# Lecanyu/SparsifyPoseGraph

Measured on AMD Instinct MI355X. Metric: nodes_marginalized_per_s, higher is better.
Workload: dtype f64

## Files before the change

### sparsifyposegraph_amd/csrc/spg_host_stream.cpp

```cpp
#include "spg_graph_impl.h"

#if defined(__x86_64__)
#include <x86intrin.h>
static inline uint64_t ticks_now() { return __rdtsc(); }
#else
static inline uint64_t ticks_now() { return (uint64_t)(now_s() * 1e9); }
#endif

namespace {
enum : uint8_t { SV_WAITING = 0, SV_STABLE = 1, SV_INFLIGHT = 2, SV_DONE = 3 };
constexpr int kStreamSlots = 2048;
constexpr int kStreamMailStride = 8;

__attribute__((always_inline)) inline void unregister_blanket(spg_graph *g, const int32_t s) {
    const spg_graph::SSlot &sl = g->sslots[s];
    spg_graph::VRec *const vr = g->vr.data();
    for (int i = 0; i < sl.nv; i++) {
        spg_graph::SVtx &sx = vr[sl.verts[i]].s;
        for (int j = 0; j < sx.nown; j++) if (sx.own[j] == s) { sx.own[j] = sx.own[--sx.nown]; break; }
    }
}

struct Streamer {
    spg_graph *g;
    const bool emulate;
    const int D, ps, rec;
    const int32_t P;
    int32_t cursor = 0;
    int32_t prefetched_to = 0;
    int32_t n_done = 0, n_inflight = 0, pending_bell = 0, bell_no = 0;
    bool fallback = false;
    int32_t cap_wait = -1;
    uint64_t t_idle = 0;

    Streamer(spg_graph *g_, bool emu) : g(g_), emulate(emu), D(g_->d), ps(g_->ps), rec(g_->rec), P((int32_t)g_->pending.size()), arena_dev(g_->dev) {}

    struct SvView { spg_graph::VRec *vr; spg_graph::SVtx &operator[](int32_t i) const { return vr[i].s; } };

    long n_exam = 0, n_park[8] = {0};
    const bool prof = [] { const char *e = getenv("SPG_STREAM_PROF"); return e && e[0] == '1'; }();
    uint64_t pt[8] = {0}, pn[8] = {0}, pt_last = 0;
    inline void P0() { if (prof) pt_last = ticks_now(); }
    inline void P1(int i) { if (prof) { const uint64_t n = ticks_now(); pt[i] += n - pt_last; pn[i]++; pt_last = n; } }
    void park(std::vector<int32_t> &heads, int32_t on, int32_t p) { g->wl_next[p] = heads[on]; heads[on] = p; }
    void wake(std::vector<int32_t> &heads, int32_t on) {
        for (int32_t p = heads[on]; p >= 0;) { const int32_t nx = g->wl_next[p]; g->s_woken.push_back(p); p = nx; }
        heads[on] = -1;
    }

    static inline int find(const int32_t *X, const int nX, const int32_t y) { for (int i = 0; i < nX; i++) if (X[i] == y) return i; return -1; }
    static inline void adj_remove(InlVec<spg_graph::AdjEnt, 7> &av, const int32_t eid) {
        for (size_t j = 0; j < av.size(); j++) if (av[j].eid == eid) { av[j] = av.back(); av.pop_back(); break; }
    }
    inline void set_pend(spg_graph::SSlot &sl, const int32_t *X, const int nX) {
        const int32_t *const cst = g->cst.data();
        sl.npend = 0;
        for (int i = 1; i < nX; i++) if (cst[X[i]] >= 0) { if (sl.npend == 3) { sl.npend = -1; break; } sl.pend[sl.npend++] = X[i]; }
    }
    __attribute__((always_inline)) inline void register_blanket(const int32_t s, const int32_t p, const int32_t *X, const int nX) {
        const SvView sv{g->vr.data()};
        spg_graph::SSlot &sl = g->sslots[s];
        sl.pos = p; sl.root = X[0]; sl.nv = nX;
        memcpy(sl.verts, X, sizeof(int32_t) * (size_t)nX);
        set_pend(sl, X, nX);
        for (int i = 0; i < nX; i++) { spg_graph::SVtx &sx = sv[X[i]]; sx.own[sx.nown++] = s; }
    }
// ... 123 lines not shown
        if (mine < 0) {
            for (int i = 0; i < nX; i++) if (sv[X[i]].nown == spg_graph::kSOwn) { park(g->wl_done, slots[sv[X[i]].own[0]].pos, p); return 0; }
            if (g->s_free.empty()) { g->wl_next[p] = cap_wait; cap_wait = p; return 0; }
        }
        if (!emulate && cell_slot[launch_seq & (uint32_t)(port.slots - 1)] != -1) { g->wl_next[p] = cap_wait; cap_wait = p; return 0; }
        const int n_new_max = k - 1, n_new_vert_max = 2 * (k - 1);
        const int64_t new_len = (int64_t)n_new_max * rec, out_len = emulate ? SPG_OUT_LEN(n_new_max, n_new_vert_max) : 0;
        if (g->used + new_len + out_len > g->cap) { fallback = true; return 0; }
        for (int i = 1; i < ne; i++) {
            const int32_t eid = E[i]; const int64_t key = edges[eid].key;
            int j = i - 1;
            for (; j >= 0 && edges[E[j]].key > key; j--) E[j + 1] = E[j];
            E[j + 1] = eid;
        }
        int32_t s = mine;
        if (s < 0) { s = g->s_free.back(); g->s_free.pop_back(); }
        spg_graph::SSlot &sl = g->sslots[s];
        if (mine < 0) register_blanket(s, p, X, nX);
        sl.ne = ne; sl.n_new_max = n_new_max; sl.logi = -1; sl.bell = bell_no + 1; sl.launched = 1;
        sl.tag = (++g->ctx->tag_counter & 0x3fffffff) + 1;
        sl.mcell = (int32_t)(launch_seq & (uint32_t)(port.slots - 1));
        if (!emulate) { cell_slot[sl.mcell] = s; launch_seq++; }
        sl.out_off = emulate ? g->used : -1;
        sl.new_off = g->used + out_len;
        g->used += new_len + out_len;
        memcpy(sl.edges, E, sizeof(int32_t) * (size_t)ne);
        cst[v] = (p << 2) | SV_INFLIGHT; sv[v].slot = s;
        P1(3);
        if (!emulate) build_packet(s, pending_bell);
        if (helper) hp.cell_tag[sl.mcell] = (uint32_t)sl.tag;
        P1(4);
        pending_bell++;
        n_inflight++;
        if (emulate) g->s_fifo.push_back(s);
        if (g->wl_stable[p] >= 0) wake(g->wl_stable, p);
        return 1;
    }

    void commit(const int32_t s, const double *recd, const bool final_seen) {
        spg_graph::SSlot &sl = g->sslots[s];
        const int32_t p = sl.pos, v = sl.root;
        const int status = (int)recd[0], inf = (int)recd[1], n_new = (int)recd[4];
        sl.logi = (int32_t)g->log.size();
        g->log.push_back({g->vid[v], sl.bell, status, inf, recd[2], recd[3]});
        g->stats.max_blanket = std::max(g->stats.max_blanket, sl.nv);
        const bool fine = (status == SPG_OK || status == SPG_ST_KLD_NOT_PD);
        if (!fine) g->stats.n_bad_status++;
        else {
            for (int i = 0; i < sl.ne; i++) {
                const int32_t eid = sl.edges[i];
                GEdge &e = g->edges[eid];
                e.alive = 0;
                adj_remove(g->vr[e.vtx[0]].adj, eid);
                if (e.vtx[1] != e.vtx[0]) adj_remove(g->vr[e.vtx[1]].adj, eid);
            }
            g->n_mutations += sl.ne + 1;
            g->n_live_e -= sl.ne;
            g->valive[v] = 0;
            g->vr[v].adj.clear();
            g->n_live_v--;
            g->stats.n_removed++;
            const int64_t key0 = g->key_base + (int64_t)p * spg_graph::kKeyStride;
            if (!emulate) {
                for_each_compact_edge(recd, n_new, [&](int e, int la, int lb) {
                    const int32_t va = sl.verts[la], vb = sl.verts[lb];
                    GEdge ge;
// ... 257 lines not shown
        std::vector<spg_blanket_desc> blk(take);
        std::vector<int64_t> vpo;
        std::vector<spg_edge_ref> er;
        std::vector<int32_t> ev;
        for (size_t t = 0; t < take; t++) {
            const spg_graph::SSlot &sl = g->sslots[fifo[live[t]]];
            spg_blanket_desc &bd = blk[t];
            append_blanket_desc(g, sl.verts, sl.nv, 1, sl.edges, sl.ne, bd, vpo, er, ev);
            bd.n_new_max = sl.n_new_max; bd.n_new_vert_max = 2 * sl.n_new_max;
            bd.new_off = sl.new_off; bd.new_len = (int64_t)sl.n_new_max * rec; bd.out_off = sl.out_off;
        }
        spg_round_desc rd{};
        rd.opts = &g->opts; rd.n_blankets = (int32_t)take; rd.first = 0; rd.count = (int32_t)take;
        rd.blankets = blk.data(); rd.vert_pose_off = vpo.data(); rd.edges = er.data(); rd.edge_vert = ev.data();
        rd.n_vert_total = (int64_t)vpo.size(); rd.n_edge_total = (int64_t)er.size(); rd.n_edge_vert_total = (int64_t)ev.size();
        rd.mail_base = 0; rd.mail_len = 0; rd.slot = 0; rd.tag = ++g->ctx->tag_counter;
        if (int r = g->ctx->be.run_round(g->ctx->be.user, g->dev, &rd)) return r;
        if (int r = g->ctx->be.synchronize(g->ctx->be.user)) return r;
        for (size_t t = 0; t < take; t++) {
            const int32_t s = fifo[live[t]];
            const spg_graph::SSlot &sl = g->sslots[s];
            const int64_t olen = SPG_OUT_LEN(sl.n_new_max, 2 * sl.n_new_max);
            if (int r = g->ctx->be.download(g->ctx->be.user, g->host.data() + sl.out_off, (char *)g->dev + sl.out_off * 8, olen)) return r;
            ready.push_back(s);
            fifo[live[t]] = -1;
        }
        while (fifo_head < fifo.size() && fifo[fifo_head] < 0) fifo_head++;
        return 0;
    }

    std::vector<int32_t> &woken = g->s_woken, &ready = g->s_ready, &fin = g->s_fin;
    size_t fin_head = 0;
    unsigned n_polls = 0;
    uint64_t last_progress = 0, idle_since = 0;

    int take_results() {
        ready.clear();
        P0();
        if (emulate) { if (int r = poll_emulated()) return r; }
        else if (n_inflight) {
            if (helper) take_helper_results(); else poll_hip((++n_polls & 15) ? 10 : 1 << 20);
        }
        P1(0);
        return 0;
    }
    void commit_ready() {
        for (size_t ri = 0; ri < ready.size(); ri++) {
            const int32_t s = ready[ri];
            const double *recd = emulate ? g->host.data() + g->sslots[s].out_off : (helper ? ready_rec[ri] : cell(s));
            const bool fin_now = emulate || (helper ? (((uint64_t)recd[5]) & 1) != 0 : mail_state(recd[5], g->sslots[s].tag) == MAIL_FINAL);
            P0();
            commit(s, recd, fin_now);
            P1(1);
        }
    }
    void examine_woken() {
        if (!fallback) {
            if (woken.size() > 1) std::sort(woken.begin(), woken.end());
            for (size_t wi = 0; wi < woken.size(); wi++) {
                examine(woken[wi]);
                if (pending_bell >= 8) ring();
            }
        }
        woken.clear();
    }
    void late_results() {
        if (emulate || !(fin.size() - fin_head >= 192 || g->s_free.size() < 256 || (cap_wait >= 0 && fin_head < fin.size()))) return;
        P0();
        const size_t n = std::min<size_t>(64, fin.size() - fin_head);
        for (size_t i = 0; i < n; i++) __builtin_prefetch((const void *)cell(fin[fin_head + i]));
        for (size_t i = 0; i < n; i++) {
            const int32_t s = fin[fin_head];
            const volatile double *c = cell(s);
            if (mail_state(c[5], g->sslots[s].tag) != MAIL_FINAL) break;
            harvest(s, (const double *)c);
            fin_head++;
        }
        if (fin_head > 8192) { fin.erase(fin.begin(), fin.begin() + (long)fin_head); fin_head = 0; }
        P1(6);
        if (!woken.empty()) {
            if (!fallback) for (size_t wi = 0; wi < woken.size(); wi++) examine(woken[wi]);
            woken.clear();
        }
    }
    void advance_cursor(const bool got) {
        if (fallback || cursor >= P) return;
        int budget = got ? 4 : 32;
        while (cursor < P && budget-- > 0 && !fallback) {
            examine(cursor++);
            if (!woken.empty()) { for (size_t wi = 0; wi < woken.size() && !fallback; wi++) examine(woken[wi]); woken.clear(); }
        }
    }
    int idle_check() {
        const uint64_t t1 = ticks_now();
        if (!idle_since) idle_since = t1;
        if (n_inflight == 0 && fin_head == fin.size()) {
            fallback = true;
            return 1;
        }
        if (((t1 - last_progress) >> 35) != 0) {
            set_err(g->ctx, SPG_EHIP, "streaming driver: no blanket completed within 10 s");
            return SPG_EHIP;
        }
        return 0;
    }
    int drain() {
        if (!emulate) {
            const double t0 = now_s();
            for (; fin_head < fin.size(); fin_head++) {
                const int32_t s = fin[fin_head];
                const volatile double *c = cell(s);
                uint32_t spins = 0;
                while (mail_state(c[5], g->sslots[s].tag) != MAIL_FINAL) {
                    if ((++spins & 0xfff) == 0 && now_s() - t0 > 10.0) { set_err(g->ctx, SPG_EHIP, "streaming driver: a blanket's KLD tail did not complete within 10 s"); return SPG_EHIP; }
                    cpu_pause();
                }
                harvest(s, (const double *)c);
            }
            woken.clear();
        }
        fin.clear();
        return 0;
    }
    void account(const uint64_t t_begin, const double s_begin) {
        if (idle_since) { t_idle += ticks_now() - idle_since; idle_since = 0; }
        const uint64_t t_end = ticks_now();
        const double secs = now_s() - s_begin;
        const double idle = (t_end > t_begin) ? secs * (double)t_idle / (double)(t_end - t_begin) : 0.0;
        g->stats.device_seconds += idle;
        g->stats.host_seconds += secs - idle;
        g->stats.schedule_seconds += secs - idle;
        if (prof) {
            const char *nm[8] = {"poll", "commit", "examine: parked", "examine: launch decision", "packet", "doorbell", "late results", "launch tail"};
            const double tps = (double)(t_end - t_begin) / secs;
            for (int i = 0; i < 8; i++) fprintf(stderr, "stream prof %-26s %8llu x %8.1f ns = %8.3f ms\n", nm[i], (unsigned long long)pn[i], pn[i] ? 1e9 * (double)pt[i] / tps / (double)pn[i] : 0.0, 1e3 * (double)pt[i] / tps);
        }
    }

    int run() {
        const uint64_t t_begin = ticks_now();
        const double s_begin = now_s();
        last_progress = t_begin;
        for (;;) {
            if (int r = take_results()) return r;
            const bool got = !ready.empty();
            if (got && idle_since) { t_idle += ticks_now() - idle_since; idle_since = 0; }
            commit_ready();
            examine_woken();
            late_results();
            advance_cursor(got);
            ring();
            if (n_done == P) break;
            if (fallback && n_inflight == 0) break;
            if (got || cursor < P) { last_progress = ticks_now(); continue; }
            if (int r = idle_check()) { if (r < 0) return r; break; }
        }
        if (int r = drain()) return r;
        account(t_begin, s_begin);
        return 0;
    }
};
}

int stream_marginalize(spg_graph *g, bool *started) {
    const spg_options &o = g->opts;
    if (started) *started = false;
    static const bool env_off = [] { const char *e = getenv("SPG_STREAM"); return e && e[0] == '0'; }();
    spg::StreamPort *const sim = g->ctx->is_hip ? nullptr : g->ctx->sim_port;
    const bool emulate = !g->ctx->is_hip && !sim;
    if (env_off || g->stream_disabled) return 1;
    if (emulate && g->stream_emulation < 0) return 1;
    if (g->nranks != 1 || o.algorithm != SPG_ALG_NFR || o.topology != SPG_TOPO_TREE || o.lin_point != SPG_LIN_GLOBAL || (o.flags & ~SPG_FLAG_NFR_FACTOR_DESCENT) != 0) return 1;
    const int32_t P = (int32_t)g->pending.size();
    if (P < (emulate ? 1 : 64)) return 1;
    Streamer S(g, emulate);
    if (sim) {
        if (sim->slots < kStreamSlots || sim->mail_stride < kStreamMailStride) return 1;
        S.port = *sim;
    } else if (!emulate) {
        int prc = spg::hip_stream_open(&g->ctx->be, g->d, kStreamSlots, kStreamMailStride, &S.port);
        if (prc < 0) { copy_backend_error(g->ctx); return prc; }
        if (prc > 0) return 1;
    }
    const size_t V = g->vid.size();
    if (g->cst.size() < V) g->cst.resize(V, -1);
    for (int32_t p = 0; p < P; p++) { g->cst[g->pending[p]] = (p << 2) | SV_WAITING; g->vr[g->pending[p]].s.nown = 0; }
    g->wl_next.assign((size_t)P, -1); g->wl_stable.assign((size_t)P, -1); g->wl_done.assign((size_t)P, -1);
    if (g->sslots.size() < (size_t)kStreamSlots) g->sslots.resize(kStreamSlots);
// ... 64 lines not shown
```

### sparsifyposegraph_amd/csrc/spg_internal.h

```cpp
#pragma once
#include <cstddef>
#include <cstdint>
#include "../../include/spg.h"

namespace spg {

int hip_backend_create(int device, spg_backend *out, char *errbuf, size_t errlen);
void hip_backend_destroy(spg_backend *b);
void *hip_backend_stream(spg_backend *b);
const char *hip_backend_error(spg_backend *b);
int hip_backend_launches(spg_backend *b);
int hip_backend_device(spg_backend *b);
void hip_backend_profile(spg_backend *b, int enable);
void hip_backend_profile_read(spg_backend *b, double *ms, double *bytes, long long *launches, long long *blankets);
void hip_backend_profile_read_worker(spg_backend *b, double *ms, double *bytes, long long *runs, long long *blankets);
void hip_backend_profile_read_big(spg_backend *b, double *ms, double *flops, long long *count, int *nmax);
void hip_backend_set_factor_descent(spg_backend *b, double rel_tol, int max_cycles);
int hip_backend_end_of_call(spg_backend *b);

constexpr int kQCap = 16384;
constexpr int kPktHdr = 13;
constexpr int kPktWords = 192;
constexpr int kPktStride = 64;
constexpr int kWorkerMaxN = 36;
constexpr int kBells = 16, kBellStride = 512;
struct WorkQ {
    unsigned long long stop;
    unsigned long long pad[7];
    unsigned long long tail[kBells * kBellStride];
    unsigned long long item[kQCap];
};

struct StreamPort {
    unsigned long long *pkt = nullptr;
    WorkQ *q = nullptr;
    unsigned long long tail = 0;
    int bells = 1;
    const double *h_mail = nullptr;
    unsigned long long d_mail = 0;
    int mail_stride = 0, slots = 0;
};
int hip_stream_open(spg_backend *b, int D, int slots, int mail_stride, StreamPort *out);
void hip_stream_close(spg_backend *b, const StreamPort *port, double alg_bytes, long long blankets);

struct BlanketVariant;
struct KArgs;
#pragma GCC visibility push(hidden)
int hip_blanket_launch(const BlanketVariant &v, void *stream, void *ev_start, void *ev_stop, const KArgs &ka, int nblocks, size_t lds_bytes,
                       char *err, size_t errlen);
int hip_worker_launch(int D, int grid, size_t lds_bytes, void *stream, void *ev_start, void *ev_stop, WorkQ *q, unsigned long long *ticket,
                      long long idle_ticks, int bells, int lazy, char *err, size_t errlen);
int hip_local_point_launch(int D, void *stream, int count, const double *arena, double *lpose, const spg_blanket_desc *blk, const int64_t *vpo,
                           const spg_edge_ref *er, const int32_t *ev, const int32_t *list, const int64_t *lp_off, int32_t *flag, char *err, size_t errlen);
#pragma GCC visibility pop

struct DenseGraphIn {
// ... 94 lines not shown
```

### sparsifyposegraph_amd/csrc/spg_kernels.hip

```cpp
#include <hip/hip_runtime.h>
#include <hip/hip_ext.h>
#include <cstdio>
#include "../../include/spg.h"
#include "spg_blanket_layout.hpp"
#include "spg_dev_geom.hpp"
#include "spg_dev_la.hpp"
#include "spg_dev_wave.hpp"
#include "spg_internal.h"

using namespace spgdev;

using spg::EC; using spg::SPG_ALG_NFR_LM; using spg::Layout; using spg::make_layout; using spg::KArgs;

namespace {

__device__ __forceinline__ int uni32(int v) { return __builtin_amdgcn_readfirstlane(v); }
__device__ __forceinline__ unsigned long long uni64(unsigned long long v) {
    unsigned lo = __builtin_amdgcn_readfirstlane((unsigned)(v & 0xffffffffu)), hi = __builtin_amdgcn_readfirstlane((unsigned)(v >> 32));
    return (unsigned long long)lo | ((unsigned long long)hi << 32);
}
template <class T>
__device__ __forceinline__ T *uniptr(T *p) { return reinterpret_cast<T *>(uni64(reinterpret_cast<unsigned long long>(p))); }

__device__ __forceinline__ int utri(int r, int c, int D) { return r * D - (r * (r - 1)) / 2 + (c - r); }
// ... 143 lines not shown
    constexpr int REC = PS + D * (D + 1) / 2;
    const int tid = threadIdx.x;
    const int nv = bd.n_vert, m = bd.n_remove, k = nv - m;
    const Layout L = make_layout(D, NT, k, m, ALG, a.topology, bd.pad_);
    const int n = L.n, nm = L.nm, ld = L.ld, ldm = L.ldm;
    double *mat = GWS ? (a.gws + (size_t)gws_slot * (size_t)a.gws_stride) : (smem + L.small_doubles);
    double *pose = smem + L.o_pose, *cs = smem + L.o_cs, *ev = smem + L.o_ev, *Sv = smem + L.o_S;
    double *w = smem + L.o_w, *ldb = smem + L.o_ldb, *Lb = smem + L.o_Lb, *nJ = smem + L.o_nJ, *X = smem + L.o_X;
    double *eJ = smem + L.o_eJ, *eO = smem + L.o_eO, *eT = smem + L.o_eT;
    int *ints = reinterpret_cast<int *>(smem + L.o_int);
    int *perm = ints + L.i_perm, *keep = ints + L.i_keep, *sorted = ints + L.i_sorted, *comp = ints + L.i_comp;
    int *pairs = ints + L.i_pairs, *echv = ints + L.i_ev, *misc = ints + L.i_misc, *pij = ints + L.i_pij;
    double *M1 = mat + L.o_M1, *M2 = mat + L.o_M2, *M3 = mat + L.o_M3, *Hmm = mat + L.o_Hmm, *Hmk = mat + L.o_Hmk;
    Team<NT> T{tid, smem + L.o_red, misc + 0};
    const bool use_wave_hw = !GWS && (n <= kWaveMax) && !((a.flags >> 17) & 1);
    const bool use_wave = use_wave_hw && (NT == 64);
    const bool split = (NT == 128) && (ALG != SPG_ALG_GLC) && use_wave_hw && !(a.flags & SPG_FLAG_FORCE_EIG);
    double *xch = smem + L.o_xch;
    double *arena = a.arena;
    double *orec = a.mail ? (a.mail + (bd.out_off - a.mail_base)) : (arena + bd.out_off);

    int status = SPG_OK, info = 0, n_new = 0;
    double kld = __builtin_nan(""), min_gap = __builtin_inf();

    bool published = false;
    double *recbuf = smem + L.o_eJ;
    double *orl = smem + L.o_eO;
    auto publish = [&]() {
        if (COH) {
            T.sync();
            const int nrec = n_new * REC;
            for (int it = tid; it < nrec; it += NT) strec<true>(arena + bd.new_off + it, recbuf[it]);
            const bool compact = (a.flags >> 20) & 1;
            if (tid == 0) {
                orl[0] = (double)status; orl[1] = (double)info; orl[2] = kld; orl[3] = min_gap; orl[4] = (double)n_new; orl[5] = 0.0;
                if (compact) {
                    unsigned long long w0 = 0, w1 = 0;
                    for (int e = 0; e < n_new; e++) {
                        const unsigned long long pr = (unsigned long long)((m + pairs[2 * e]) & 15) | ((unsigned long long)((m + pairs[2 * e + 1]) & 15) << 4);
                        if (e < 8) w0 |= pr << (8 * e); else w1 |= pr << (8 * (e - 8));
                    }
                    orl[6] = __longlong_as_double((long long)w0); orl[7] = __longlong_as_double((long long)w1);
                } else
                for (int e = 0; e < n_new; e++) {
                    orl[SPG_OUT_HDR + 4 * e + 0] = (double)SPG_EDGE_BINARY;
                    orl[SPG_OUT_HDR + 4 * e + 1] = (double)(e * REC);
                    orl[SPG_OUT_HDR + 4 * e + 2] = (double)REC;
                    orl[SPG_OUT_HDR + 4 * e + 3] = 2.0;
                    orl[SPG_OUT_HDR + 4 * bd.n_new_max + 2 * e + 0] = (double)(m + pairs[2 * e]);
                    orl[SPG_OUT_HDR + 4 * bd.n_new_max + 2 * e + 1] = (double)(m + pairs[2 * e + 1]);
                }
            }
            wait_stores();
            T.sync();
            const int olen = compact ? 8 : SPG_OUT_HDR + 4 * bd.n_new_max + 2 * n_new;
            if (tid < 64) {
                for (int t = tid; t < olen; t += 64) if (t != 5) strec<true>(orec + t, orl[t]);
                wait_stores();
                if (tid == 0) {
                    __hip_atomic_store(&orec[5], SPG_READY_WORD(a.tag), __ATOMIC_RELAXED, __HIP_MEMORY_SCOPE_SYSTEM);
                    orl[5] = (double)wall_clock64();
                }
            }
            published = true;
            return;
        }
        T.sync();
        if (tid == 0) {
            orec[0] = (double)status; orec[1] = (double)info; orec[2] = kld; orec[3] = min_gap; orec[4] = (double)n_new;
            for (int e = 0; e < n_new; e++) {
                orec[SPG_OUT_HDR + 4 * e + 0] = (double)SPG_EDGE_BINARY;
                orec[SPG_OUT_HDR + 4 * e + 1] = (double)(e * REC);
                orec[SPG_OUT_HDR + 4 * e + 2] = (double)REC;
                orec[SPG_OUT_HDR + 4 * e + 3] = 2.0;
                orec[SPG_OUT_HDR + 4 * bd.n_new_max + 2 * e + 0] = (double)(m + pairs[2 * e]);
                orec[SPG_OUT_HDR + 4 * bd.n_new_max + 2 * e + 1] = (double)(m + pairs[2 * e + 1]);
            }
        }
        __threadfence_system();
        T.sync();
        if (tid == 0) {
            __hip_atomic_store(&orec[5], SPG_READY_WORD(a.tag), __ATOMIC_RELEASE, __HIP_MEMORY_SCOPE_SYSTEM);
        }
        published = true;
    };
    auto finish = [&]() {
        if (!published) publish();
        else if (tid == 0) { strec<COH>(orec + 2, kld); strec<COH>(orec + 0, (double)status); }
        if (tid == 0) {
            if (COH) { wait_stores(); __hip_atomic_store(&orec[5], SPG_FINAL_WORD(a.tag), __ATOMIC_RELAXED, __HIP_MEMORY_SCOPE_SYSTEM); }
            else { __threadfence_system(); __hip_atomic_store(&orec[5], SPG_FINAL_WORD(a.tag), __ATOMIC_RELEASE, __HIP_MEMORY_SCOPE_SYSTEM); }
        }
    };
    const bool stamping = ((a.flags >> 16) & 1) && bd.tinfo_off >= 0;
    auto STAMP = [&](int idx) {
        if (stamping) {
            T.sync();
            if (tid == 0) arena[bd.tinfo_off + idx] = (double)__builtin_amdgcn_s_memtime();
        }
    };
    auto CSTAMP = [&](int idx) {
        if (stamping) {
            if (!split) { T.sync(); if (tid == 0) arena[bd.tinfo_off + idx] = (double)__builtin_amdgcn_s_memtime(); }
            else if ((tid & 63) == 0) arena[bd.tinfo_off + idx] = (double)__builtin_amdgcn_s_memtime();
        }
    };
    STAMP(0);
    if (tid == 0) { misc[0] = 0; misc[1] = 0; misc[2] = 0; misc[6] = 0; misc[7] = 0; misc[8] = 0; misc[9] = 0; }
    for (int v = tid; v < nv; v += NT) {
        const double *p = arena + bvpo[v];
        if (D == 6) iso_from_tq(p, pose + v * PSZ);
        else { pose[v * PSZ] = p[0]; pose[v * PSZ + 1] = p[1]; pose[v * PSZ + 2] = p[2]; }
    }
    for (int i = tid; i < n * ld; i += NT) M1[i] = 0.0;
    for (int i = tid; i < nm * ldm; i += NT) Hmm[i] = 0.0;
    for (int i = tid; i < nm * ld; i += NT) Hmk[i] = 0.0;
    T.sync();
    STAMP(23);
    if (bd.n_edge == 0 || m < 1) { status = SPG_ST_EMPTY_BLANKET; finish(); return; }
    constexpr bool is_glc = (ALG == SPG_ALG_GLC);
    constexpr bool has_lm = (ALG == SPG_ALG_NFR_LM);
    if (is_glc && !(a.topology == SPG_TOPO_DENSE || a.topology == SPG_TOPO_TREE)) {
        status = SPG_ST_UNSUPPORTED;
        finish(); return;
    }

    int lm_left = 0;
    if (a.lin_point != SPG_LIN_GLOBAL && !(m > 1 && k < 2)) {
        if (is_glc) { status = SPG_ST_UNSUPPORTED; finish(); return; }
        if (n < nv || m != 1) { status = SPG_ST_NEEDS_LOCAL_OPTIMIZATION; finish(); return; }
        int *cntv = perm;
        for (int v = tid; v < nv; v += NT) cntv[v] = 0;
        T.sync();
        for (int e = tid; e < bd.n_edge; e += NT) {
            const spg_edge_ref er = ber[e];
            if (er.kind != SPG_EDGE_BINARY) { misc[8] = 1; continue; }
            int vi = bev[er.vbegin], vj = bev[er.vbegin + 1];
            if (vi != 0) atomicAdd(&cntv[vi], 1);
            if (vj != 0) atomicAdd(&cntv[vj], 1);
        }
        T.sync();
        for (int v = 1 + tid; v < nv; v += NT) if (cntv[v] > 1) misc[9] = 1;
        T.sync();
        if (misc[8] || n < nv || (misc[9] && m != 1)) { status = SPG_ST_NEEDS_LOCAL_OPTIMIZATION; finish(); return; }
        if (misc[9]) {
            if constexpr (has_lm) lm_left = 10;
            else { status = SPG_ST_NEEDS_LOCAL_OPTIMIZATION; finish(); return; }
        } else {
        if (tid == 0) {
// ... 30 lines not shown
                    pose[vi * PSZ + 2] = normalize_theta(-rec[2]);
                }
            }
        }
        }
        T.sync();
    }
    auto hadd = [&](int R, int Cc, double val) {
        if (R < nm) {
            if (Cc < nm) Hmm[R * ldm + Cc] += val;
            else Hmk[R * ld + (Cc - nm)] += val;
        } else if (Cc >= nm) {
            M1[(R - nm) * ld + (Cc - nm)] += val;
        }
    };
    double *eE = nJ;
    double *bnew = ev, *bcur = Sv, *xs = cs, *pbak = smem + L.o_Ng;
    double lm_lambda = 0, lm_ni = 2, lm_chi = 0, lm_scale = 0;
    int lm_it = 0, lm_q = 0, lm_phase = 0;
    bool lm_redo = false;
    for (;;) {
    if (has_lm && (lm_left > 0 || lm_redo)) {
        if (lm_phase > 0 || lm_redo) {
            for (int i = tid; i < n * ld; i += NT) M1[i] = 0.0;
            for (int i = tid; i < nm * ldm; i += NT) Hmm[i] = 0.0;
            for (int i = tid; i < nm * ld; i += NT) Hmk[i] = 0.0;
        }
        for (int i = tid; i < n; i += NT) bnew[i] = 0.0;
        if (tid == 0) xch[0] = 0.0;
        T.sync();
    }
    for (int base = 0; base < bd.n_edge; base += EC) {
        int cnt = min(EC, bd.n_edge - base);
        if (tid < cnt) {
            const spg_edge_ref er = ber[base + tid];
            int vi = 0, vj = 0;
            if (er.kind == SPG_EDGE_BINARY) {
                vi = bev[er.vbegin]; vj = bev[er.vbegin + 1];
                double rec[PS];
#pragma unroll
                for (int i = 0; i < PS; i++) rec[i] = ldrec<COH>(arena + er.off + i);
                if (D == 6) {
                    double Z[kIso];
                    iso_from_tq(rec, Z);
                    se3_edge_jac(pose + vi * PSZ, pose + vj * PSZ, Z, eJ + tid * 2 * DD, eJ + tid * 2 * DD + DD, (has_lm && lm_left > 0) ? eE + tid * D : nullptr);
                } else {
                    se2_edge_jac(pose + vi * PSZ, pose + vj * PSZ, rec, eJ + tid * 2 * DD, eJ + tid * 2 * DD + DD, (has_lm && lm_left > 0) ? eE + tid * D : nullptr);
                }
            } else {
                if (!is_glc) misc[1] = 1;
                vi = -1;
            }
            echv[2 * tid] = vi; echv[2 * tid + 1] = vj;
        }
        for (int it = tid; it < cnt * DD; it += NT) {
            int e = it / DD, rc = it - e * DD, r = rc / D, c = rc - r * D;
            const spg_edge_ref er = ber[base + e];
            int lo = r < c ? r : c, hi = r < c ? c : r;
            eO[it] = (er.kind == SPG_EDGE_BINARY) ? ldrec<COH>(arena + er.off + PS + utri(lo, hi, D)) : 0.0;
        }
        T.sync();
        STAMP(24);
        for (int it = tid; it < cnt * 2 * DD; it += NT) {
            int e = it / (2 * DD), rem = it - e * 2 * DD, wch = rem / DD, rc = rem - wch * DD, r = rc / D, c = rc - r * D;
            const double *J = eJ + e * 2 * DD + wch * DD, *Om = eO + e * DD;
            double s = 0;
#pragma unroll
            for (int p = 0; p < D; p++) s += Om[r * D + p] * J[p * D + c];
            eT[it] = s;
        }
        T.sync();
        STAMP(25);
        if (has_lm && lm_left > 0) {
            {
                double c2 = 0;
                for (int it = tid; it < cnt * D; it += NT) {
                    int e = it / D, p = it - e * D;
                    if (echv[2 * e] < 0) continue;
                    const double *Om = eO + e * DD, *er_ = eE + e * D;
                    double sacc = 0;
#pragma unroll
                    for (int q = 0; q < D; q++) sacc += Om[p * D + q] * er_[q];
                    c2 += er_[p] * sacc;
                }
                c2 = T.sum(c2);
                if (tid == 0) xch[0] += c2;
                for (int e = 0; e < cnt; e++) {
                    if (echv[2 * e] < 0) continue;
                    for (int side = 0; side < 2; side++) {
                        const int v = echv[2 * e + side];
                        if (tid < D && v >= 1) {
                            const double *Te = eT + e * 2 * DD + side * DD, *er_ = eE + e * D;
// ... 447 lines not shown
        } else {
            chol_lower(TT, M3, n, ld, Sv);
            CSTAMP(14);
            bool fail = ((*TT.flag) != 0);
            TT.sync();
            if (TT.tid == 0) { (*TT.flag) = 0; }
            TT.sync();
            if (!fail) {
                double ldC = chol_logdet(TT, M3, n, ld);
                CSTAMP(15);
                tri_inverse_lower(TT, M3, M2, n, ld, Sv);
                CSTAMP(16);
                int sh = ceil_log2(n), tot = n << sh;
                double f2 = 0;
                for (int it = TT.tid; it < tot; it += TT.size) {
                    int i = it >> sh, j = it & ((1 << sh) - 1);
                    if (j <= i) {
                        double s = 0;
                        for (int q = i; q < n; q++) s += M2[q * ld + i] * M2[q * ld + j];
                        M3[i * ld + j] = s;
                        M3[j * ld + i] = s;
                        f2 += (i == j) ? s * s : 2.0 * s * s;
                    }
                }
                double fro2 = TT.sum(f2);
                if (fro2 < 5e4 * 5e4 && isfinite(fro2)) {
                    if (TT.tid == 0) { xch[0] = 1.0; xch[1] = -ldC; }
                }
            }
        }
    };
    if (tid == 0) { xch[0] = 0.0; xch[1] = 0.0; }
    T.sync();
    {
        int st_ = SPG_OK;
        if (split) {
            Team<64> S{tid & 63, nullptr, misc + ((tid < 64) ? 6 : 2)};
            if (tid < 64) { int s2 = chow_liu_tree(S); if (S.tid == 0) misc[7] = s2; }
            else gauge_chain(S);
            T.sync();
            st_ = misc[7];
            min_gap = (k > 2) ? cs[0] : min_gap;
        } else {
            st_ = chow_liu_tree(T);
            if (st_ == SPG_OK && !(a.flags & SPG_FLAG_FORCE_EIG)) gauge_chain(T);
        }
        if (st_ != SPG_OK) { status = st_; finish(); return; }
        T.sync();
        if (xch[0] != 0.0) { gauge_ok = true; logdetS = xch[1]; Sg = M3; Scr = M1; }
        T.sync();
        if (tid == 0) { misc[0] = 0; misc[2] = 0; misc[6] = 0; }
        T.sync();
    }
    STAMP(9);
    if (stop_after == 3) { finish(); return; }
    for (int e = tid; e < ne; e += NT) {
        int va = m + pairs[2 * e], vb = m + pairs[2 * e + 1];
        double *rec = arena + bd.new_off + (int64_t)e * REC;
        if (D == 6) {
            double Z[kIso], q[4];
            iso_inv_mul(pose + va * PSZ, pose + vb * PSZ, Z);
            R_to_quat(Z, q);
            double *rw = COH ? (recbuf + e * REC) : rec;
            rw[0] = Z[9]; rw[1] = Z[10]; rw[2] = Z[11]; rw[3] = q[0]; rw[4] = q[1]; rw[5] = q[2]; rw[6] = q[3];
            se3_edge_jac(pose + va * PSZ, pose + vb * PSZ, Z, nJ + e * 2 * DD, nJ + e * 2 * DD + DD, nullptr);
        } else {
            double z[3];
            se2_between(pose + va * PSZ, pose + vb * PSZ, z);
            double *rw = COH ? (recbuf + e * REC) : rec;
            rw[0] = z[0]; rw[1] = z[1]; rw[2] = z[2];
            se2_edge_jac(pose + va * PSZ, pose + vb * PSZ, z, nJ + e * 2 * DD, nJ + e * 2 * DD + DD, nullptr);
        }
    }
    T.sync();
    if (ne == 1) {
        for (int it = tid; it < 2 * DD; it += NT) if (fabs(nJ[it]) < 2.220446049250313e-16) nJ[it] = 0.0;
        T.sync();
    }

    STAMP(10);
    if (stop_after == 4) { finish(); return; }
    if (!gauge_ok) {
        for (int it = tid; it < n * ld; it += NT) M3[it] = M1[it];
        T.sync();
        if (!jacobi_eigh<NT>(T, M3, M2, n, ld, cs)) { status = SPG_ST_EIG_FAIL; finish(); return; }
        for (int i = tid; i < n; i += NT) ev[i] = M3[i * ld + i];
        T.sync();
        if (stop_after == 5) { finish(); return; }
        sort_ascending<NT>(T, ev, 1, n, perm);
        {
            double cnt = 0;
            for (int i = tid; i < n; i += NT) cnt += (ev[i] < 1e-5) ? 1.0 : 0.0;
            int smalleigs = (int)T.sum(cnt);
            if (smalleigs <= D) {
                for (int j = tid; j < r; j += NT) { int idx = perm[D + j]; keep[j] = idx; Sv[j] = 1.0 / ev[idx]; }
            } else {
                info |= SPG_INFO_RANK_DEFICIENT;
                if (tid == 0) {
                    double *nrm = cs;
                    for (int c = 0; c < smalleigs; c++) {
                        int col = perm[c];
                        double s2 = 0;
                        for (int e = 0; e < ne; e++) {
                            int oa = pairs[2 * e] * D, ob = pairs[2 * e + 1] * D;
                            const double *Ja = nJ + e * 2 * DD, *Jb = Ja + DD;
                            for (int rr = 0; rr < D; rr++) {
// ... 274 lines not shown
        if (D == 3) { P[0] = 0; P[1] = 0; P[2] = 0; }
        else { P[0] = 0; P[1] = 0; P[2] = 0; P[3] = 0; P[4] = 0; P[5] = 0; P[6] = 1; }
        for (int e = 0; e < bd.n_edge; e++) {
            const spg_edge_ref r = er[bd.edge_begin + e];
            const int vi = ev[r.vbegin], vj = ev[r.vbegin + 1];
            if (vi == 0 && vj == 0) continue;
            const double *z = arena + r.off;
            if (D == 3) {
                if (vi == 0) {
                    const double c = cos(P[2]), sn = sin(P[2]);
                    double *o = P + vj * 3;
                    o[0] = P[0] + c * z[0] - sn * z[1]; o[1] = P[1] + sn * z[0] + c * z[1]; o[2] = normalize_theta(P[2] + z[2]);
                } else {
                    const double cz = cos(z[2]), sz = sin(z[2]);
                    const double zi[3] = {-(cz * z[0] + sz * z[1]), -(-sz * z[0] + cz * z[1]), normalize_theta(-z[2])};
                    const double *a = P + vj * 3;
                    const double c = cos(a[2]), sn = sin(a[2]);
                    const double ox = a[0] + c * zi[0] - sn * zi[1], oy = a[1] + sn * zi[0] + c * zi[1], ot = normalize_theta(a[2] + zi[2]);
                    double *o = P + vi * 3;
                    o[0] = ox; o[1] = oy; o[2] = ot;
                }
            } else {
                double zq[7], out[7];
                for (int i = 0; i < 7; i++) zq[i] = z[i];
                { const double nn = 1.0 / sqrt(zq[3] * zq[3] + zq[4] * zq[4] + zq[5] * zq[5] + zq[6] * zq[6]); for (int i = 3; i < 7; i++) zq[i] *= nn; }
                if (vi == 0) { tq_compose(P, zq, out); for (int i = 0; i < 7; i++) P[vj * 7 + i] = out[i]; }
                else { double zi[7]; tq_inverse(zq, zi); tq_compose(P + vj * 7, zi, out); for (int i = 0; i < 7; i++) P[vi * 7 + i] = out[i]; }
            }
        }
    }
    flag[blockIdx.x] = ok ? 1 : 0;
}

using spg::kQCap; using spg::kPktHdr; using spg::kPktWords; using spg::kPktStride; using spg::kWorkerMaxN; using spg::kBells; using spg::kBellStride;
using spg::WorkQ;

__device__ __forceinline__ unsigned long long load_sys(const unsigned long long *p) {
    return __hip_atomic_load(p, __ATOMIC_RELAXED, __HIP_MEMORY_SCOPE_SYSTEM);
}


template <int D, int ALG>
__global__ void __launch_bounds__(128) blanket_worker(WorkQ *q, unsigned long long *ticket, long long idle_ticks, int n_bells, int lazy) {
    extern __shared__ double smem[];
    __shared__ unsigned long long pk[kPktWords];
    __shared__ unsigned long long s_item;
    const int tid = threadIdx.x;
    for (;;) {
        if (tid == 0) {
            const unsigned long long my = atomicAdd(ticket, 1ULL);
            unsigned long long it = 0;
            long long t0 = wall_clock64();
            unsigned long long seen = ~0ULL;
            for (;;) {
                const unsigned long long tail = load_sys(&q->tail[(blockIdx.x % n_bells) * kBellStride]);
                if (tail > my) { it = load_sys(&q->item[my % kQCap]); break; }
                if (load_sys(&q->stop)) break;
                if (tail != seen) { seen = tail; t0 = wall_clock64(); }
                else if (wall_clock64() - t0 > idle_ticks) break;
                const unsigned long long ahead = my - tail;
                if (lazy) {
                    if (ahead >= 2) for (int z = 0; z < lazy; z++) __builtin_amdgcn_s_sleep(32);
                } else {
                    if (ahead >= 64) __builtin_amdgcn_s_sleep(64);
                    else if (ahead >= 4) __builtin_amdgcn_s_sleep(8);
                }
            }
            s_item = it;
        }
        __syncthreads();
        const unsigned long long it = s_item;
        if (!it) return;
        const long long t_pick = wall_clock64();
        const unsigned long long *gp = reinterpret_cast<const unsigned long long *>(it);
        if (tid < kPktStride) pk[tid] = load_sys(gp + tid);
        __syncthreads();
        const int n_words = (int)(uni64(pk[12]) & 0xffffffffu);
        for (int w = kPktStride + tid; w < n_words && w < kPktWords; w += 128) pk[w] = load_sys(gp + w);
        __syncthreads();
        unsigned long long h[kPktHdr];
#pragma unroll
        for (int w = 0; w < kPktHdr; w++) h[w] = uni64(pk[w]);
        KArgs a;
        a.arena = reinterpret_cast<double *>(h[0]);
        a.mail = reinterpret_cast<double *>(h[1]);
        a.mail_base = (int64_t)h[2];
        a.blk = nullptr; a.vpo = nullptr; a.er = nullptr; a.ev = nullptr; a.list = nullptr; a.gws = nullptr; a.gws_stride = 0;
        a.algorithm = ALG == SPG_ALG_GLC ? SPG_ALG_GLC : SPG_ALG_NFR;
        a.topology = (int)(h[9] & 0xffffffffu); a.flags = (int)(h[9] >> 32);
        a.lin_point = (int)(h[10] & 0xffffffffu); a.tag = (int)(h[10] >> 32);
        a.chord_ratio = __longlong_as_double((long long)h[11]);
        spg_blanket_desc bd;
        bd.vert_begin = 0; bd.edge_begin = 0;
        bd.out_off = (int64_t)h[3]; bd.new_off = (int64_t)h[4]; bd.tinfo_off = (int64_t)h[5]; bd.new_len = 0;
        bd.n_vert = (int)(h[6] & 0xffffffffu); bd.n_remove = (int)(h[6] >> 32);
        bd.n_edge = (int)(h[7] & 0xffffffffu); bd.n_new_max = (int)(h[7] >> 32);
        bd.n_new_vert_max = (int)(h[8] & 0xffffffffu); bd.pad_ = (int)(h[8] >> 32);
        const int64_t *vpo = reinterpret_cast<const int64_t *>(pk + kPktHdr);
        const spg_edge_ref *er = reinterpret_cast<const spg_edge_ref *>(pk + kPktHdr + bd.n_vert);
        const int32_t *ev = reinterpret_cast<const int32_t *>(pk + kPktHdr + bd.n_vert + 3 * bd.n_edge);
        const long long t_body = wall_clock64();
        blanket_body<D, 128, false, ALG, true>(a, bd, vpo, er, ev, 0, smem);
        __syncthreads();
        if ((h[12] >> 32) & 0x40000000u) {
            if (tid == 0 && a.mail) {
                double *orec = a.mail + (bd.out_off - a.mail_base);
                const double *orl_ = smem + make_layout(D, 128, bd.n_vert - bd.n_remove, bd.n_remove, ALG, a.topology, bd.pad_).o_eO;
                orec[3] = (double)((long long)orl_[5] - t_pick) + 1e-6 * (double)(wall_clock64() - t_pick);
                __threadfence_system();
            }
        }
// ... 76 lines not shown
```

Before: 3.047 million.

## Overlap kernel loads, parallelize result publish, and refine host idle accounting

The worker kernel now loads the whole packet in one pass with two loads per lane, dropping a dependent second round and a barrier. Edge records for the first chunk are prefetched into registers early and staged in shared memory, so their global latency overlaps pose setup. New-edge measurements and Jacobians are computed by the Chow-Liu team while the other team runs the gauge chain. The output header is written by 64 lanes in parallel instead of a single thread. Host idle accounting is reworked to count only turns with no progress and reuses the tick read, which adds profiling output but has little speed intent.

```diff
diff --git a/sparsifyposegraph_amd/csrc/spg_host_stream.cpp b/sparsifyposegraph_amd/csrc/spg_host_stream.cpp
--- a/sparsifyposegraph_amd/csrc/spg_host_stream.cpp
+++ b/sparsifyposegraph_amd/csrc/spg_host_stream.cpp
@@ -31,7 +31,8 @@
     int32_t n_done = 0, n_inflight = 0, pending_bell = 0, bell_no = 0;
     bool fallback = false;
     int32_t cap_wait = -1;
-    uint64_t t_idle = 0;
+    uint64_t t_idle = 0, n_wait_turns = 0;
+    uint32_t n_launched = 0;
 
     Streamer(spg_graph *g_, bool emu) : g(g_), emulate(emu), D(g_->d), ps(g_->ps), rec(g_->rec), P((int32_t)g_->pending.size()), arena_dev(g_->dev) {}
 
@@ -221,6 +222,7 @@
         P1(4);
         pending_bell++;
         n_inflight++;
+        n_launched++;
         if (emulate) g->s_fifo.push_back(s);
         if (g->wl_stable[p] >= 0) wake(g->wl_stable, p);
         return 1;
@@ -544,7 +546,7 @@
     std::vector<int32_t> &woken = g->s_woken, &ready = g->s_ready, &fin = g->s_fin;
     size_t fin_head = 0;
     unsigned n_polls = 0;
-    uint64_t last_progress = 0, idle_since = 0;
+    uint64_t last_progress = 0;
 
     int take_results() {
         ready.clear();
@@ -603,9 +605,7 @@
             if (!woken.empty()) { for (size_t wi = 0; wi < woken.size() && !fallback; wi++) examine(woken[wi]); woken.clear(); }
         }
     }
-    int idle_check() {
-        const uint64_t t1 = ticks_now();
-        if (!idle_since) idle_since = t1;
+    int idle_check(const uint64_t t1) {
         if (n_inflight == 0 && fin_head == fin.size()) {
             fallback = true;
             return 1;
@@ -635,7 +635,6 @@
         return 0;
     }
     void account(const uint64_t t_begin, const double s_begin) {
-        if (idle_since) { t_idle += ticks_now() - idle_since; idle_since = 0; }
         const uint64_t t_end = ticks_now();
         const double secs = now_s() - s_begin;
         const double idle = (t_end > t_begin) ? secs * (double)t_idle / (double)(t_end - t_begin) : 0.0;
@@ -646,6 +645,8 @@
             const char *nm[8] = {"poll", "commit", "examine: parked", "examine: launch decision", "packet", "doorbell", "late results", "launch tail"};
             const double tps = (double)(t_end - t_begin) / secs;
             for (int i = 0; i < 8; i++) fprintf(stderr, "stream prof %-26s %8llu x %8.1f ns = %8.3f ms\n", nm[i], (unsigned long long)pn[i], pn[i] ? 1e9 * (double)pt[i] / tps / (double)pn[i] : 0.0, 1e3 * (double)pt[i] / tps);
+            fprintf(stderr, "stream prof %-26s %8llu x %8.1f ns = %8.3f ms of %.3f ms\n", "waiting for the device", (unsigned long long)n_wait_turns,
+                    n_wait_turns ? 1e9 * (double)t_idle / tps / (double)n_wait_turns : 0.0, 1e3 * (double)t_idle / tps, 1e3 * secs);
         }
     }
 
@@ -653,19 +654,24 @@
         const uint64_t t_begin = ticks_now();
         const double s_begin = now_s();
         last_progress = t_begin;
+        uint64_t t_turn = t_begin;
         for (;;) {
+            const uint32_t launched0 = n_launched;
+            const int32_t cursor0 = cursor;
             if (int r = take_results()) return r;
             const bool got = !ready.empty();
-            if (got && idle_since) { t_idle += ticks_now() - idle_since; idle_since = 0; }
             commit_ready();
             examine_woken();
             late_results();
             advance_cursor(got);
             ring();
+            const uint64_t t_now = ticks_now();
+            if (!got && n_launched == launched0 && cursor == cursor0) { t_idle += t_now - t_turn; n_wait_turns++; }
+            t_turn = t_now;
             if (n_done == P) break;
             if (fallback && n_inflight == 0) break;
-            if (got || cursor < P) { last_progress = ticks_now(); continue; }
-            if (int r = idle_check()) { if (r < 0) return r; break; }
+            if (got || cursor < P) { last_progress = t_now; continue; }
+            if (int r = idle_check(t_now)) { if (r < 0) return r; break; }
         }
         if (int r = drain()) return r;
         account(t_begin, s_begin);
diff --git a/sparsifyposegraph_amd/csrc/spg_internal.h b/sparsifyposegraph_amd/csrc/spg_internal.h
--- a/sparsifyposegraph_amd/csrc/spg_internal.h
+++ b/sparsifyposegraph_amd/csrc/spg_internal.h
@@ -21,7 +21,6 @@
 constexpr int kQCap = 16384;
 constexpr int kPktHdr = 13;
 constexpr int kPktWords = 192;
-constexpr int kPktStride = 64;
 constexpr int kWorkerMaxN = 36;
 constexpr int kBells = 16, kBellStride = 512;
 struct WorkQ {
diff --git a/sparsifyposegraph_amd/csrc/spg_kernels.hip b/sparsifyposegraph_amd/csrc/spg_kernels.hip
--- a/sparsifyposegraph_amd/csrc/spg_kernels.hip
+++ b/sparsifyposegraph_amd/csrc/spg_kernels.hip
@@ -199,35 +199,41 @@
             const int nrec = n_new * REC;
             for (int it = tid; it < nrec; it += NT) strec<true>(arena + bd.new_off + it, recbuf[it]);
             const bool compact = (a.flags >> 20) & 1;
-            if (tid == 0) {
-                orl[0] = (double)status; orl[1] = (double)info; orl[2] = kld; orl[3] = min_gap; orl[4] = (double)n_new; orl[5] = 0.0;
-                if (compact) {
-                    unsigned long long w0 = 0, w1 = 0;
-                    for (int e = 0; e < n_new; e++) {
-                        const unsigned long long pr = (unsigned long long)((m + pairs[2 * e]) & 15) | ((unsigned long long)((m + pairs[2 * e + 1]) & 15) << 4);
-                        if (e < 8) w0 |= pr << (8 * e); else w1 |= pr << (8 * (e - 8));
-                    }
-                    orl[6] = __longlong_as_double((long long)w0); orl[7] = __longlong_as_double((long long)w1);
-                } else
-                for (int e = 0; e < n_new; e++) {
-                    orl[SPG_OUT_HDR + 4 * e + 0] = (double)SPG_EDGE_BINARY;
-                    orl[SPG_OUT_HDR + 4 * e + 1] = (double)(e * REC);
-                    orl[SPG_OUT_HDR + 4 * e + 2] = (double)REC;
-                    orl[SPG_OUT_HDR + 4 * e + 3] = 2.0;
-                    orl[SPG_OUT_HDR + 4 * bd.n_new_max + 2 * e + 0] = (double)(m + pairs[2 * e]);
-                    orl[SPG_OUT_HDR + 4 * bd.n_new_max + 2 * e + 1] = (double)(m + pairs[2 * e + 1]);
-                }
-            }
-            wait_stores();
-            T.sync();
             const int olen = compact ? 8 : SPG_OUT_HDR + 4 * bd.n_new_max + 2 * n_new;
             if (tid < 64) {
-                for (int t = tid; t < olen; t += 64) if (t != 5) strec<true>(orec + t, orl[t]);
-                wait_stores();
-                if (tid == 0) {
-                    __hip_atomic_store(&orec[5], SPG_READY_WORD(a.tag), __ATOMIC_RELAXED, __HIP_MEMORY_SCOPE_SYSTEM);
-                    orl[5] = (double)wall_clock64();
-                }
+                const double h_status = (double)uni32(status), h_info = (double)uni32(info), h_nnew = (double)uni32(n_new);
+                const double h_kld = __longlong_as_double((long long)uni64((unsigned long long)__double_as_longlong(kld)));
+                const double h_gap = __longlong_as_double((long long)uni64((unsigned long long)__double_as_longlong(min_gap)));
+                const int nn0 = uni32(n_new);
+                for (int t = tid; t < olen; t += 64) {
+                    if (t == 5) continue;
+                    double val = 0.0;
+                    bool have = true;
+                    if (t < 5) val = (t == 0) ? h_status : (t == 1) ? h_info : (t == 2) ? h_kld : (t == 3) ? h_gap : h_nnew;
+                    else if (compact) {
+                        unsigned long long wv = 0;
+                        const int e0 = (t == 6) ? 0 : 8;
+                        for (int e = e0; e < nn0 && e < e0 + 8; e++) {
+                            const unsigned long long pr = (unsigned long long)((m + pairs[2 * e]) & 15) | ((unsigned long long)((m + pairs[2 * e + 1]) & 15) << 4);
+                            wv |= pr << (8 * (e - e0));
+                        }
+                        val = __longlong_as_double((long long)wv);
+                    } else if (t < SPG_OUT_HDR + 4 * bd.n_new_max) {
+                        const int e = (t - SPG_OUT_HDR) >> 2, j = (t - SPG_OUT_HDR) & 3;
+                        have = e < nn0;
+                        val = (j == 0) ? (double)SPG_EDGE_BINARY : (j == 1) ? (double)(e * REC) : (j == 2) ? (double)REC : 2.0;
+                    } else {
+                        const int q = t - (SPG_OUT_HDR + 4 * bd.n_new_max);
+                        val = (double)(m + pairs[q]);
+                    }
+                    if (have) strec<true>(orec + t, val);
+                }
+            }
+            wait_stores();
+            T.sync();
+            if (tid == 0) {
+                __hip_atomic_store(&orec[5], SPG_READY_WORD(a.tag), __ATOMIC_RELAXED, __HIP_MEMORY_SCOPE_SYSTEM);
+                orl[5] = (double)wall_clock64();
             }
             published = true;
             return;
@@ -274,6 +280,22 @@
     };
     STAMP(0);
     if (tid == 0) { misc[0] = 0; misc[1] = 0; misc[2] = 0; misc[6] = 0; misc[7] = 0; misc[8] = 0; misc[9] = 0; }
+    constexpr bool kStageRec = (ALG != SPG_ALG_NFR_LM);
+    constexpr int kStageMax = (EC * REC + NT - 1) / NT;
+    const int n_stage = kStageRec ? min(EC, bd.n_edge) * REC : 0;
+    double srec[kStageMax];
+    if (kStageRec) {
+#pragma unroll
+        for (int j = 0; j < kStageMax; j++) {
+            const int it = tid + j * NT;
+            srec[j] = 0.0;
+            if (it < n_stage) {
+                const int e = it / REC;
+                const spg_edge_ref er = ber[e];
+                if (er.kind == SPG_EDGE_BINARY) srec[j] = ldrec<COH>(arena + er.off + (it - e * REC));
+            }
+        }
+    }
     for (int v = tid; v < nv; v += NT) {
         const double *p = arena + bvpo[v];
         if (D == 6) iso_from_tq(p, pose + v * PSZ);
@@ -282,6 +304,10 @@
     for (int i = tid; i < n * ld; i += NT) M1[i] = 0.0;
     for (int i = tid; i < nm * ldm; i += NT) Hmm[i] = 0.0;
     for (int i = tid; i < nm * ld; i += NT) Hmk[i] = 0.0;
+    if (kStageRec) {
+#pragma unroll
+        for (int j = 0; j < kStageMax; j++) if (tid + j * NT < n_stage) eT[tid + j * NT] = srec[j];
+    }
     T.sync();
     STAMP(23);
     if (bd.n_edge == 0 || m < 1) { status = SPG_ST_EMPTY_BLANKET; finish(); return; }
@@ -378,6 +404,7 @@
     }
     for (int base = 0; base < bd.n_edge; base += EC) {
         int cnt = min(EC, bd.n_edge - base);
+        const bool staged = kStageRec && base == 0;
         if (tid < cnt) {
             const spg_edge_ref er = ber[base + tid];
             int vi = 0, vj = 0;
@@ -385,7 +412,7 @@
                 vi = bev[er.vbegin]; vj = bev[er.vbegin + 1];
                 double rec[PS];
 #pragma unroll
-                for (int i = 0; i < PS; i++) rec[i] = ldrec<COH>(arena + er.off + i);
+                for (int i = 0; i < PS; i++) rec[i] = staged ? eT[tid * REC + i] : ldrec<COH>(arena + er.off + i);
                 if (D == 6) {
                     double Z[kIso];
                     iso_from_tq(rec, Z);
@@ -403,7 +430,8 @@
             int e = it / DD, rc = it - e * DD, r = rc / D, c = rc - r * D;
             const spg_edge_ref er = ber[base + e];
             int lo = r < c ? r : c, hi = r < c ? c : r;
-            eO[it] = (er.kind == SPG_EDGE_BINARY) ? ldrec<COH>(arena + er.off + PS + utri(lo, hi, D)) : 0.0;
+            const int ow = PS + utri(lo, hi, D);
+            eO[it] = (er.kind == SPG_EDGE_BINARY) ? (staged ? eT[e * REC + ow] : ldrec<COH>(arena + er.off + ow)) : 0.0;
         }
         T.sync();
         STAMP(24);
@@ -917,11 +945,35 @@
     };
     if (tid == 0) { xch[0] = 0.0; xch[1] = 0.0; }
     T.sync();
+    auto new_edge_skeleton = [&](const int t0, const int stride) {
+        for (int e = t0; e < ne; e += stride) {
+            int va = m + pairs[2 * e], vb = m + pairs[2 * e + 1];
+            double *rec = arena + bd.new_off + (int64_t)e * REC;
+            if (D == 6) {
+                double Z[kIso], q[4];
+                iso_inv_mul(pose + va * PSZ, pose + vb * PSZ, Z);
+                R_to_quat(Z, q);
+                double *rw = COH ? (recbuf + e * REC) : rec;
+                rw[0] = Z[9]; rw[1] = Z[10]; rw[2] = Z[11]; rw[3] = q[0]; rw[4] = q[1]; rw[5] = q[2]; rw[6] = q[3];
+                se3_edge_jac(pose + va * PSZ, pose + vb * PSZ, Z, nJ + e * 2 * DD, nJ + e * 2 * DD + DD, nullptr);
+            } else {
+                double z[3];
+                se2_between(pose + va * PSZ, pose + vb * PSZ, z);
+                double *rw = COH ? (recbuf + e * REC) : rec;
+                rw[0] = z[0]; rw[1] = z[1]; rw[2] = z[2];
+                se2_edge_jac(pose + va * PSZ, pose + vb * PSZ, z, nJ + e * 2 * DD, nJ + e * 2 * DD + DD, nullptr);
+            }
+        }
+    };
     {
         int st_ = SPG_OK;
         if (split) {
             Team<64> S{tid & 63, nullptr, misc + ((tid < 64) ? 6 : 2)};
-            if (tid < 64) { int s2 = chow_liu_tree(S); if (S.tid == 0) misc[7] = s2; }
+            if (tid < 64) {
+                int s2 = chow_liu_tree(S);
+                if (S.tid == 0) misc[7] = s2;
+                if (s2 == SPG_OK && stop_after != 3) new_edge_skeleton(S.tid, 64);
+            }
             else gauge_chain(S);
             T.sync();
             st_ = misc[7];
@@ -939,24 +991,7 @@
     }
     STAMP(9);
     if (stop_after == 3) { finish(); return; }
-    for (int e = tid; e < ne; e += NT) {
-        int va = m + pairs[2 * e], vb = m + pairs[2 * e + 1];
-        double *rec = arena + bd.new_off + (int64_t)e * REC;
-        if (D == 6) {
-            double Z[kIso], q[4];
-            iso_inv_mul(pose + va * PSZ, pose + vb * PSZ, Z);
-            R_to_quat(Z, q);
-            double *rw = COH ? (recbuf + e * REC) : rec;
-            rw[0] = Z[9]; rw[1] = Z[10]; rw[2] = Z[11]; rw[3] = q[0]; rw[4] = q[1]; rw[5] = q[2]; rw[6] = q[3];
-            se3_edge_jac(pose + va * PSZ, pose + vb * PSZ, Z, nJ + e * 2 * DD, nJ + e * 2 * DD + DD, nullptr);
-        } else {
-            double z[3];
-            se2_between(pose + va * PSZ, pose + vb * PSZ, z);
-            double *rw = COH ? (recbuf + e * REC) : rec;
-            rw[0] = z[0]; rw[1] = z[1]; rw[2] = z[2];
-            se2_edge_jac(pose + va * PSZ, pose + vb * PSZ, z, nJ + e * 2 * DD, nJ + e * 2 * DD + DD, nullptr);
-        }
-    }
+    if (!split) new_edge_skeleton(tid, NT);
     T.sync();
     if (ne == 1) {
         for (int it = tid; it < 2 * DD; it += NT) if (fabs(nJ[it]) < 2.220446049250313e-16) nJ[it] = 0.0;
@@ -1297,7 +1332,7 @@
     flag[blockIdx.x] = ok ? 1 : 0;
 }
 
-using spg::kQCap; using spg::kPktHdr; using spg::kPktWords; using spg::kPktStride; using spg::kWorkerMaxN; using spg::kBells; using spg::kBellStride;
+using spg::kQCap; using spg::kPktHdr; using spg::kPktWords;using spg::kWorkerMaxN; using spg::kBells; using spg::kBellStride;
 using spg::WorkQ;
 
 __device__ __forceinline__ unsigned long long load_sys(const unsigned long long *p) {
@@ -1338,10 +1373,13 @@
         if (!it) return;
         const long long t_pick = wall_clock64();
         const unsigned long long *gp = reinterpret_cast<const unsigned long long *>(it);
-        if (tid < kPktStride) pk[tid] = load_sys(gp + tid);
-        __syncthreads();
-        const int n_words = (int)(uni64(pk[12]) & 0xffffffffu);
-        for (int w = kPktStride + tid; w < n_words && w < kPktWords; w += 128) pk[w] = load_sys(gp + w);
+        static_assert(kPktWords > 128 && kPktWords <= 256, "two loads per lane cover a packet slot");
+        {
+            const unsigned long long w0 = load_sys(gp + tid);
+            const unsigned long long w1 = (tid + 128 < kPktWords) ? load_sys(gp + tid + 128) : 0ULL;
+            pk[tid] = w0;
+            if (tid + 128 < kPktWords) pk[tid + 128] = w1;
+        }
         __syncthreads();
         unsigned long long h[kPktHdr];
 #pragma unroll
```

New measurement: 3.116 million, median of 6. 2.3% higher.
